# HumanCompatibleAI/imitation

Measured on AMD Instinct MI355X. Metric: env-steps/sec (gen+disc round) GAIL HalfCheetah n_envs=1024, higher is better.
Workload: dtype f32

## Files before the change

imitation_amd/csrc/policy.hip:

```cpp
#include "common.h"
#include "rn_common.h"
#include <algorithm>
#include <type_traits>
#include <cstring>

#include "../../include/imitation_hip.h"
#include "policy_common.h"

namespace {


template <int H>
struct Lds {
  static constexpr int XS = MAXD + 1, HS = H + 1, AS = MAXA + 1;
  static constexpr int x = 0;
  static constexpr int a1 = x + ROWS * XS;
  static constexpr int a2 = a1 + ROWS * HS;
  static constexpr int dz = a2 + ROWS * HS;
  static constexpr int out = dz + ROWS * HS;
  static constexpr int dout = out + ROWS * AS;
  static constexpr int aux = dout + ROWS * AS;
  static constexpr int total = aux + ROWS * AS + 64;
};

// ... 1446 lines not shown
        tr(o.pW1, H, D); tr(o.pW2, H, H); tr(o.vW1, H, D); tr(o.vW2, H, H);
        Pt[dst] = pn;
      }
    }
  }
  if (next_batch > 0 && !stats_block) {
    __syncthreads();
    prepare_stats(d, obs, adv, next_idx, next_batch, T, n_envs, update_norm, nm, nv, ncount, w.advstat, lds);
  }
}

struct CLds {
  static constexpr int RS = 68;
  static constexpr int x = 0;
  static constexpr int a1 = x + MAXD * RS;
  static constexpr int a2 = a1 + 2 * 32 * RS;
  static constexpr int dz2 = a2 + 2 * 32 * RS;
  static constexpr int dz1 = dz2 + 2 * 32 * RS;
  static constexpr int dout = dz1 + 2 * 32 * RS;
  static constexpr int aux = dout + MAXA * RS;
  static constexpr int misc = aux + MAXA * RS;
  static constexpr int scratch = misc + 8 * RS;
  static constexpr int total = scratch + 64;
};


#ifndef IA_UPD_TSTR
#define IA_UPD_TSTR 36
#endif
constexpr int UPD_TSTR = IA_UPD_TSTR;
__host__ __device__ inline int upd_tbase(int off) { return (off * UPD_TSTR + 31) >> 5; }
__host__ __device__ inline int upd_pt4(int P4) { return (upd_tbase(P4) + 3) & ~3; }

template <bool SMALL>
__device__ __forceinline__ void chain_stage_rows(const ia_policy_desc& d, const float* __restrict__ nm,
                                                 const float* __restrict__ nv, const int i0, const int row_lim,
                                                 float* __restrict__ lds, const float* __restrict__ stg, const int tw,
                                                 const int q, const int lane) {
  using L = CLds;
  const int D = d.obs_dim;
  const int S1 = (D + 3) >> 2;
#ifndef IA_SMALL_STAGE_ASIDE
#define IA_SMALL_STAGE_ASIDE 1
#endif
  constexpr int QS = (SMALL && IA_SMALL_STAGE_ASIDE) ? 1 : 0;
  const bool idle = SMALL && q != QS;
  if (!idle) {
    const int rbase = SMALL ? 0 : q * 16;
    const int l128 = lane + 64 * tw;
    const int s1r = (65536 + S1 - 1) / S1;
    for (int g = l128; g < 16 * S1; g += 128) {
      const int r = (g * s1r) >> 16, k0 = (g - r * S1) * 4;
      const bool rok = (i0 + rbase + r) < row_lim;
      float raw[4], mu[4], vr[4];
      {
        const f32x4 rq = *reinterpret_cast<const f32x4*>(stg + UpdStage::x + (rbase * S1 + g) * 4);
        const f32x4 mq = *reinterpret_cast<const f32x4*>(nm + k0);
        const f32x4 vq = *reinterpret_cast<const f32x4*>(nv + k0);
#pragma unroll
        for (int j = 0; j < 4; ++j) {
          raw[j] = rq[j];
          mu[j] = mq[j];
          vr[j] = vq[j];
        }
      }
#pragma unroll
      for (int j = 0; j < 4; ++j) {
        const bool ok = rok && k0 + j < D;
        const bool nrm = ok && d.has_norm;
        lds[L::x + (k0 + j) * L::RS + rbase + r] = ok ? (nrm ? (raw[j] - mu[j]) * vr[j] : raw[j]) : 0.f;
      }
    }
    if (tw == 0) {
      for (int e = lane; e < 16 * MAXA; e += 64) {
        lds[L::dout + (e >> 4) * L::RS + rbase + (e & 15)] = 0.f;
        lds[L::aux + (e >> 4) * L::RS + rbase + (e & 15)] = 0.f;
      }
    } else {
      for (int e = lane; e < 16 * 8; e += 64) lds[L::misc + (e >> 4) * L::RS + rbase + (e & 15)] = 0.f;
    }
  }
}

template <int KS1, bool LOCAL, bool SMALL = false, bool STAGED = false, bool TSPLIT = false>
__device__ __forceinline__ void mfma32_minibatch_chain(
    const ia_policy_desc& d, const float* __restrict__ nm, const float* __restrict__ nv, const float adv_mean,
    const float adv_std, const MbRows rows, const int i0_in, const int row_lim, const int normalize_adv, const float clip,
    const float ent_coef, const float vf_coef, float* __restrict__ slab_g, float* __restrict__ statpart,
    float* __restrict__ lds_in, const float* __restrict__ sP_in, float* __restrict__ stg_in,
    const int opaque_zero, long long* __restrict__ tstamp, const unsigned ll_seq, const bool ll_xcd = false,
    const int split_tw = 0) {
  static_assert(!TSPLIT || (!LOCAL && !SMALL && STAGED), "one tower per workgroup: several gradient workgroups only");
  float* __restrict__ lds = lds_in + opaque_zero;
  const float* __restrict__ stg = stg_in + opaque_zero;
  float* __restrict__ slab = LOCAL ? stg_in + opaque_zero + UpdStage::x : slab_g;
  unsigned long long* __restrict__ slab64 = reinterpret_cast<unsigned long long*>(slab_g);
  auto put = [&](float* p, float v) {
    if constexpr (LOCAL) *p = v;
    else if (ll_xcd) ll_store_xcd(slab64 + (p - slab), v, ll_seq);
    else ll_store_agent(slab64 + (p - slab), v, ll_seq);
  };
  const int batch = rows.batch;
  constexpr int H = 32;
  using L = CLds;
#define IA_TS(slot) do { if (tstamp && i0_in == 0 && threadIdx.x == 0) tstamp[slot] = clock64(); } while (0)
  const int tid = threadIdx.x + opaque_zero, lane = tid & 63;
  const int wv = __builtin_amdgcn_readfirstlane(tid >> 6);
  const int tw = TSPLIT ? split_tw : (SMALL ? (wv & 1) : (wv >> 2)), q = SMALL ? (wv >> 1) : (wv & 3);
  const bool helper = TSPLIT && wv >= 4;
  const int li = lane & 15, lk = lane >> 4;
  const int D = d.obs_dim, A = d.act_dim;
  const PolOff o = pol_offsets(D, A, H, d.discrete);
  const int i0 = i0_in;
  const int aw = d.discrete ? 1 : A;
  const float invB = 1.f / (float)batch;
  const int S1 = (D + 3) >> 2;
  const int oW1 = tw ? o.vW1 : o.pW1, ob1 = tw ? o.vb1 : o.pb1, oW2 = tw ? o.vW2 : o.pW2, ob2 = tw ? o.vb2 : o.pb2;
  const float* __restrict__ sP = sP_in + opaque_zero;
  const float* __restrict__ sPt = sP + ((o.total + 3) & ~3);
  constexpr int TS_ = UPD_TSTR;
  const int tW1 = upd_tbase(oW1), tW2 = upd_tbase(oW2);
  IA_TS(0);

  const int lrow = q * 16 + (lane & 15);
  const bool valid = (i0 + lrow) < row_lim;
  float r_oldlp = 0.f, r_adv = 0.f, r_ret = 0.f, r_act[4] = {0.f, 0.f, 0.f, 0.f};
  constexpr bool HANDOVER = SMALL;
  if (helper) {
  } else if (tw == 0) {
    r_oldlp = stg[UpdStage::oldlp + lrow];
    if constexpr (!HANDOVER) r_adv = stg[UpdStage::adv + lrow];
#pragma unroll
    for (int j = 0; j < 4; ++j) r_act[j] = stg[UpdStage::act + lrow * aw + min(4 * (lane >> 4) + j, aw - 1)];
  } else {
    r_ret = stg[UpdStage::ret + lrow];
    if constexpr (HANDOVER) r_adv = stg[UpdStage::adv + lrow];
  }
  float* gconst = lds + L::scratch + 32;

  IA_TS(9);
  const bool idle = (SMALL && q > 0) || helper;
  if constexpr (!STAGED) chain_stage_rows<SMALL>(d, nm, nv, i0, row_lim, lds, stg, tw, q, lane);
  IA_TS(10);
  constexpr int KT1 = KS1 / 4;
  float fW1[KT1][2][4], fW2[2][2][4], fW2T[2][2][4], fHead[2][4], fHeadT[2][4], b1c[2][4], b2c[2][4], hb[4];
  const int head_base = tw == 0 ? o.aW + min(li, A - 1) * H : o.cW;
  float c_ivar[4] = {1.f, 1.f, 1.f, 1.f}, c_logsd[4] = {0.f, 0.f, 0.f, 0.f};
  if (!helper) {
#pragma unroll
  for (int kt = 0; kt < KT1; ++kt) {
    if (4 * kt < S1) {
#pragma unroll
      for (int t = 0; t < 2; ++t)
#pragma unroll
        for (int r = 0; r < 4; ++r) fW1[kt][t][r] = sPt[tW1 + min(16 * kt + 4 * lk + r, D - 1) * TS_ + 16 * t + li];
    } else {
#pragma unroll
      for (int t = 0; t < 2; ++t)
#pragma unroll
        for (int r = 0; r < 4; ++r) fW1[kt][t][r] = 0.f;
    }
  }
#pragma unroll
  for (int t = 0; t < 2; ++t)
#pragma unroll
    for (int r = 0; r < 4; ++r) b1c[t][r] = sP[ob1 + 16 * t + 4 * lk + r];
  float my_sd = sP[o.log_std + min(lane, A - 1)];
  __builtin_amdgcn_sched_barrier(0);
#pragma unroll
  for (int kt = 0; kt < KT1; ++kt)
#pragma unroll
    for (int t = 0; t < 2; ++t)
#pragma unroll
      for (int r = 0; r < 4; ++r) fW1[kt][t][r] = (16 * kt + 4 * lk + r < D) ? fW1[kt][t][r] : 0.f;
  if constexpr (HANDOVER) {
    if (tw != 0) {
      if (!idle) {
        float advn = r_adv;
        if (normalize_adv && batch > 1) advn = (advn - adv_mean) / (adv_std + 1e-8f);
        if (lk == 0) stg_in[opaque_zero + UpdStage::adv + lrow] = advn;
      }
      if (q == 0 && !d.discrete) {
        const float sd = expf(my_sd);
        const float my_ivar = lane < A ? 1.f / (sd * sd) : 1.f;
        const float my_logsd = lane < A ? logf(sd) : 0.f;
        if (lane < 16) {
          gconst[lane] = my_ivar;
          gconst[16 + lane] = my_logsd;
        }
      }
    }
  } else {
    float my_ivar = 1.f, my_logsd = 0.f;
    if (tw == 0 && !d.discrete) {
      const float sd = expf(my_sd);
      my_ivar = lane < A ? 1.f / (sd * sd) : 1.f;
      my_logsd = lane < A ? logf(sd) : 0.f;
    }
#pragma unroll
    for (int j = 0; j < 4; ++j) {
      c_ivar[j] = __shfl(my_ivar, 4 * lk + j, 64);
      c_logsd[j] = __shfl(my_logsd, 4 * lk + j, 64);
    }
  }
  }
  IA_TS(11);
  __syncthreads();
  IA_TS(1);

  float* a1t = lds + L::a1 + tw * 32 * L::RS;
  float* a2t = lds + L::a2 + tw * 32 * L::RS;
  float* dz2t = lds + L::dz2 + tw * 32 * L::RS;
  float* dz1t = lds + L::dz1 + tw * 32 * L::RS;
  const int trow = 4 * lk * L::RS + q * 16 + li;
  auto xchg16 = [](float v, float& a, float& b) {
    const auto p2 = __builtin_amdgcn_permlane16_swap(__float_as_uint(v), __float_as_uint(v), false, false);
    a = __uint_as_float(p2[0]);
    b = __uint_as_float(p2[1]);
  };
  auto xchg32 = [](float v, float& a, float& b) {
    const auto p2 = __builtin_amdgcn_permlane32_swap(__float_as_uint(v), __float_as_uint(v), false, false);
    a = __uint_as_float(p2[0]);
    b = __uint_as_float(p2[1]);
  };
  auto group_sum = [&](float v) {
    float a, b;
    xchg16(v, a, b);
    v = a + b;
    xchg32(v, a, b);
    return a + b;
  };
  auto group_max = [&](float v) {
    float a, b;
    xchg16(v, a, b);
    v = fmaxf(a, b);
    xchg32(v, a, b);
    return fmaxf(a, b);
  };
  if (!idle) {
  f32x4 a1[2], a2[2];
  {
    f32x4 acc[2][2] = {{{b1c[0][0], b1c[0][1], b1c[0][2], b1c[0][3]}, {0.f, 0.f, 0.f, 0.f}},
                       {{b1c[1][0], b1c[1][1], b1c[1][2], b1c[1][3]}, {0.f, 0.f, 0.f, 0.f}}};
    float xb[KT1][4];
#pragma unroll
    for (int kt = 0; kt < KT1; ++kt)
#pragma unroll
      for (int r = 0; r < 4; ++r) xb[kt][r] = lds[L::x + min(16 * kt + 4 * lk + r, MAXD - 1) * L::RS + q * 16 + li];
    if (HANDOVER && tw == 0) {
      r_adv = stg_in[opaque_zero + UpdStage::adv + lrow];
#pragma unroll
      for (int j = 0; j < 4; ++j) {
        c_ivar[j] = gconst[4 * lk + j];
        c_logsd[j] = gconst[16 + 4 * lk + j];
      }
    }
    __builtin_amdgcn_sched_barrier(0);
#pragma unroll
    for (int kt = 0; kt < KT1; ++kt)
      if (4 * kt < S1) {
#pragma unroll
        for (int r = 0; r < 4; ++r) {
          acc[0][kt & 1] = mfma16(fW1[kt][0][r], xb[kt][r], acc[0][kt & 1]);
          acc[1][kt & 1] = mfma16(fW1[kt][1][r], xb[kt][r], acc[1][kt & 1]);
        }
      }
#pragma unroll
    for (int kt = 0; kt < 2; ++kt)
#pragma unroll
      for (int r = 0; r < 4; ++r)
#pragma unroll
        for (int t = 0; t < 2; ++t) fW2[kt][t][r] = sPt[tW2 + (16 * kt + 4 * lk + r) * TS_ + 16 * t + li];
#pragma unroll
    for (int t = 0; t < 2; ++t)
#pragma unroll
      for (int r = 0; r < 4; ++r) b2c[t][r] = sP[ob2 + 16 * t + 4 * lk + r];
#pragma unroll
    for (int t = 0; t < 2; ++t)
#pragma unroll
      for (int r = 0; r < 4; ++r) {
        a1[t][r] = fast_tanh(acc[t][0][r] + acc[t][1][r]);
        a1t[trow + (16 * t + r) * L::RS] = a1[t][r];
      }
  }
  IA_TS(2);
  {
    f32x4 acc[2][2] = {{{b2c[0][0], b2c[0][1], b2c[0][2], b2c[0][3]}, {0.f, 0.f, 0.f, 0.f}},
                       {{b2c[1][0], b2c[1][1], b2c[1][2], b2c[1][3]}, {0.f, 0.f, 0.f, 0.f}}};
#pragma unroll
    for (int kt = 0; kt < 2; ++kt)
#pragma unroll
      for (int r = 0; r < 4; ++r) {
        acc[0][kt] = mfma16(fW2[kt][0][r], a1[kt][r], acc[0][kt]);
        acc[1][kt] = mfma16(fW2[kt][1][r], a1[kt][r], acc[1][kt]);
      }
    {
      const bool head_on = tw == 0 ? li < A : li == 0;
      float hraw[2][4], braw[4];
#pragma unroll
      for (int kt = 0; kt < 2; ++kt)
#pragma unroll
        for (int r = 0; r < 4; ++r) hraw[kt][r] = sP[head_base + 16 * kt + 4 * lk + r];
#pragma unroll
      for (int r = 0; r < 4; ++r) braw[r] = sP[tw == 0 ? o.ab + min(4 * lk + r, A - 1) : o.cb];
      __builtin_amdgcn_sched_barrier(0);
#pragma unroll
      for (int kt = 0; kt < 2; ++kt)
#pragma unroll
        for (int r = 0; r < 4; ++r) fHead[kt][r] = head_on ? hraw[kt][r] : 0.f;
#pragma unroll
      for (int r = 0; r < 4; ++r) hb[r] = (tw == 0 && 4 * lk + r >= A) ? 0.f : braw[r];
    }
#pragma unroll
    for (int t = 0; t < 2; ++t)
#pragma unroll
      for (int r = 0; r < 4; ++r) {
        a2[t][r] = fast_tanh(acc[t][0][r] + acc[t][1][r]);
        a2t[trow + (16 * t + r) * L::RS] = a2[t][r];
      }
  }
  IA_TS(3);
  float hout[4];
  {
    f32x4 acc[2] = {{hb[0], hb[1], hb[2], hb[3]}, {0.f, 0.f, 0.f, 0.f}};
#pragma unroll
    for (int kt = 0; kt < 2; ++kt)
#pragma unroll
      for (int r = 0; r < 4; ++r) acc[kt] = mfma16(fHead[kt][r], a2[kt][r], acc[kt]);
#pragma unroll
    for (int r = 0; r < 4; ++r) hout[r] = acc[0][r] + acc[1][r];
  }
  IA_TS(4);
#pragma unroll
  for (int kt = 0; kt < 2; ++kt)
#pragma unroll
    for (int t = 0; t < 2; ++t)
#pragma unroll
      for (int r = 0; r < 4; ++r) fW2T[kt][t][r] = sP[oW2 + (16 * kt + 4 * lk + r) * H + 16 * t + li];
#pragma unroll
  for (int t = 0; t < 2; ++t)
#pragma unroll
    for (int r = 0; r < 4; ++r)
      fHeadT[t][r] = sP[tw == 0 ? o.aW + min(4 * lk + r, A - 1) * H + 16 * t + li : o.cW + 16 * t + 4 * lk + r];
  float dout[4] = {0.f, 0.f, 0.f, 0.f}, dvb = 0.f;
  if (tw == 0) {
    float logp = 0.f, entropy = 0.f, lse = 0.f;
    int act_i = 0;
    if (d.discrete) act_i = (int)r_act[0];
    IA_TS(12);
    if (!d.discrete) {
#pragma unroll
      for (int j = 0; j < 4; ++j)
        if (4 * lk + j < A) {
          const float diff = r_act[j] - hout[j];
          logp += -(diff * diff) * (0.5f * c_ivar[j]) - c_logsd[j] - LOG_SQRT_2PI;
          entropy += 0.5f + LOG_SQRT_2PI + c_logsd[j];
        }
      logp = group_sum(logp);
      entropy = group_sum(entropy);
    } else {
      float mx = -3.0e38f, o_act = 0.f;
#pragma unroll
      for (int j = 0; j < 4; ++j)
        if (4 * lk + j < A) {
          mx = fmaxf(mx, hout[j]);
          o_act += (4 * lk + j == act_i) ? hout[j] : 0.f;
        }
      mx = group_max(mx);
      o_act = group_sum(o_act);
      float se = 0.f;
#pragma unroll
      for (int j = 0; j < 4; ++j)
        if (4 * lk + j < A) se += expf(hout[j] - mx);
      lse = mx + logf(group_sum(se));
      logp = o_act - lse;
#pragma unroll
      for (int j = 0; j < 4; ++j)
        if (4 * lk + j < A) {
          const float l = hout[j] - lse;
          entropy -= expf(l) * l;
        }
      entropy = group_sum(entropy);
    }
    IA_TS(13);
    float advn = r_adv;
    if constexpr (!HANDOVER)
      if (normalize_adv && batch > 1) advn = (advn - adv_mean) / (adv_std + 1e-8f);
    const float log_ratio = logp - r_oldlp;
    const float ratio = expf(log_ratio);
    const float lo = 1.f - clip, hi = 1.f + clip;
    const float pl1 = advn * ratio;
    const float pl2 = advn * fminf(fmaxf(ratio, lo), hi);
    const float g1 = pl1 < pl2 ? 1.f : (pl1 == pl2 ? 0.5f : 0.f);
    const float g2 = pl2 < pl1 ? 1.f : (pl1 == pl2 ? 0.5f : 0.f);
    const float inrange = (ratio >= lo && ratio <= hi) ? 1.f : 0.f;
    const float dlogp = valid ? -invB * advn * (g1 + g2 * inrange) * ratio : 0.f;
    IA_TS(14);
    float* doutrow = lds + L::dout + lrow;
    float* auxrow = lds + L::aux + lrow;
    if (!d.discrete) {
#pragma unroll
      for (int j = 0; j < 4; ++j)
        if (4 * lk + j < A) {
          const float diff = r_act[j] - hout[j];
          dout[j] = dlogp * diff * c_ivar[j];
          doutrow[(4 * lk + j) * L::RS] = dout[j];
          auxrow[(4 * lk + j) * L::RS] = valid ? dlogp * (diff * diff * c_ivar[j] - 1.f) - ent_coef * invB : 0.f;
        }
    } else {
#pragma unroll
      for (int j = 0; j < 4; ++j)
        if (4 * lk + j < A) {
          const float l = hout[j] - lse, p = expf(l);
          const float dH = -p * (l + entropy);
          float g = dlogp * ((4 * lk + j == act_i ? 1.f : 0.f) - p);
          g += valid ? -ent_coef * invB * dH : 0.f;
          dout[j] = g;
          doutrow[(4 * lk + j) * L::RS] = g;
        }
    }
    if (lk == 0) {
      float* mrow = lds + L::misc + lrow;
      mrow[2 * L::RS] = valid ? -fminf(pl1, pl2) : 0.f;
      mrow[3 * L::RS] = valid ? -entropy : 0.f;
      mrow[4 * L::RS] = valid ? (ratio - 1.f) - log_ratio : 0.f;
      mrow[5 * L::RS] = valid ? (fabsf(ratio - 1.f) > clip ? 1.f : 0.f) : 0.f;
    }
    IA_TS(15);
  } else {
    const float v = __shfl(hout[0], li, 64);
    const float verr = r_ret - v;
    dvb = valid ? vf_coef * 2.f * (v - r_ret) * invB : 0.f;
    if (lk == 0) {
      lds[L::misc + 1 * L::RS + lrow] = dvb;
      lds[L::misc + 6 * L::RS + lrow] = valid ? verr * verr : 0.f;
    }
  }
  IA_TS(5);
  f32x4 dz2[2];
  if (tw == 0) {
    f32x4 acc[2] = {{0.f, 0.f, 0.f, 0.f}, {0.f, 0.f, 0.f, 0.f}};
#pragma unroll
    for (int r = 0; r < 4; ++r)
      if (r < A) {
        const bool on = 4 * lk + r < A;
        acc[0] = mfma16(on ? fHeadT[0][r] : 0.f, dout[r], acc[0]);
        acc[1] = mfma16(on ? fHeadT[1][r] : 0.f, dout[r], acc[1]);
      }
#pragma unroll
    for (int t = 0; t < 2; ++t)
#pragma unroll
      for (int r = 0; r < 4; ++r) dz2[t][r] = acc[t][r] * (1.f - a2[t][r] * a2[t][r]);
  } else {
#pragma unroll
    for (int t = 0; t < 2; ++t)
#pragma unroll
      for (int r = 0; r < 4; ++r) dz2[t][r] = fHeadT[t][r] * dvb * (1.f - a2[t][r] * a2[t][r]);
  }
#pragma unroll
  for (int t = 0; t < 2; ++t)
#pragma unroll
    for (int r = 0; r < 4; ++r) dz2t[trow + (16 * t + r) * L::RS] = dz2[t][r];
  {
    f32x4 acc[2][2] = {{{0.f, 0.f, 0.f, 0.f}, {0.f, 0.f, 0.f, 0.f}}, {{0.f, 0.f, 0.f, 0.f}, {0.f, 0.f, 0.f, 0.f}}};
#pragma unroll
    for (int kt = 0; kt < 2; ++kt)
#pragma unroll
      for (int r = 0; r < 4; ++r) {
        acc[0][kt] = mfma16(fW2T[kt][0][r], dz2[kt][r], acc[0][kt]);
// ... 2077 lines not shown
      if (tid == 0) ll_store_agent(sq64 + (seq_out & 1u) * 64 + bid, part, seq_out);
    }
    EP_TS(2);
    if (have_next) stage_rows(bnext);
    if (tid < 64) {
      const u64* wp = sq64 + (seq_out & 1u) * 64 + min(tid, nwg - 1);
      u64 t;
      unsigned it = 0;
      for (;;) {
        t = __hip_atomic_load(wp, __ATOMIC_RELAXED, __HIP_MEMORY_SCOPE_AGENT);
        if (__all((unsigned)(t >> 32) == seq_out)) break;
        if (timed_out(it)) { fail = true; break; }
      }
      s_part[tid] = tid < nwg ? __uint_as_float((unsigned)t) : 0.f;
    }
    if (__any(fail) && lane == 0) s_fail = 1;
    __syncthreads();
    if (s_fail) return;
    EP_TS(3);
    float total_sq = 0.f;
    for (int q = 0; q < nwg; ++q) total_sq += s_part[q];
    const float total_norm = sqrtf(total_sq);
    const float coef = fminf(max_norm / (total_norm + 1e-6f), 1.0f);
    {
      const float step_size = st.step_size[k], bc2_sqrt = st.bc2_sqrt[k];
      u64* dst = par64 + (long long)(seq_out & 1u) * o.total;
#pragma unroll
      for (int j = 0; j < NPC; ++j) {
        const int i = i0 + tid + j * NT;
        if (i < i1) {
          const float gi = g[j] * coef;
          const float mi = m_[j] + (gi - m_[j]) * (1.f - beta1);
          const float vi = v_[j] * beta2 + (1.f - beta2) * gi * gi;
          const float denom = sqrtf(vi) / bc2_sqrt + eps;
          const float pn = p_[j] - step_size * (mi / denom);
          ll_store_agent(dst + i, pn, seq_out);
          p_[j] = pn;
          m_[j] = mi;
          v_[j] = vi;
        }
      }
    }
    if (bid == 0 && stats != nullptr) {
      __shared__ float s_st[5];
      if (tid >= 64 && tid < 69) {
        const int kk = tid - 64;
        float sv = 0.f;
        for (int q = 0; q < nblk; ++q) sv += s_stat[q * 8 + kk];
        sv *= 1.f / (float)b;
        stats[(long long)mb * 8 + kk] = sv;
        s_st[kk] = sv;
      }
      __syncthreads();
      if (tid == 0) {
        stats[(long long)mb * 8 + 5] = s_st[0] + ent_coef * s_st[2] + vf_coef * s_st[1];
        stats[(long long)mb * 8 + 6] = total_norm;
        stats[(long long)mb * 8 + 7] = coef;
      }
    }
    EP_TS(4);
  }
  tid = threadIdx.x;
#pragma unroll
  for (int j = 0; j < NPC; ++j) {
    const int i = bid * chunk + tid + j * NT;
    if (i < min(o.total, (bid + 1) * chunk)) {
      m[i] = m_[j];
      v[i] = v_[j];
      P[i] = p_[j];
      int dst = i;
      auto tr = [&](int b0, int rows_, int cols) {
        if (i >= b0 && i < b0 + rows_ * cols) {
          const int r = (i - b0) / cols, cc = (i - b0) % cols;
          dst = b0 + cc * rows_ + r;
        }
      };
      tr(o.pW1, H, D); tr(o.pW2, H, H); tr(o.vW1, H, D); tr(o.vW2, H, H);
      Pt[dst] = p_[j];
    }
  }
#undef EP_TS
}

template <int NPT, bool TIMING, int KS1, bool LOCAL, bool SHARD, bool SMALL, bool TSPLIT, int OWNER>
__device__ __forceinline__ void ppo_update_body(
    const ia_policy_desc& d, float* __restrict__ P, float* __restrict__ Pt, float* __restrict__ m, float* __restrict__ v,
    float* __restrict__ nm, float* __restrict__ nv, int32_t* __restrict__ ncount, int update_norm,
    const float* __restrict__ obs, const float* __restrict__ actions, const float* __restrict__ old_logp,
    const float* __restrict__ adv, const float* __restrict__ ret, const int64_t* __restrict__ perm, int T, int n_envs,
    int normalize_adv, float clip, float ent_coef, float vf_coef, float max_norm, float beta1, float beta2, float eps,
    float* __restrict__ ws, int nblk, int n_slices, float* __restrict__ stats, UpdSched sch, int xcd_pack,
    long long* __restrict__ tstamp ,
    ShardArgs sh) {
  constexpr int H = 32;
  using L = CLds;
  extern __shared__ float lds_raw[];
  float* lds = lds_raw + (((16u - (__builtin_amdgcn_groupstaticsize() & 15u)) & 15u) >> 2);
  __shared__ int s_ok, s_pub, s_fail, s_pubw[4];
  if (!TIMING) tstamp = nullptr;
  long long tacc[12] = {0, 0, 0, 0, 0, 0, 0, 0, 0, 0, 0, 0};
  long long tprev = 0, tend = 0;
#define UPD_TS(k) do { if (tstamp && tid == 0) { const long long tn = wall_clock64(); tacc[k] += tn - tprev; tprev = tn; } } while (0)
  if (xcd_pack && (blockIdx.x & 7)) return;
  const int vb = xcd_pack ? blockIdx.x >> 3 : blockIdx.x;
  static_assert(!TSPLIT || (!LOCAL && !SHARD && !SMALL), "one tower per workgroup: several gradient workgroups, one process");
  static_assert(OWNER == 0 || (OWNER == 1 && TSPLIT), "slices by tower: the tower-split form only");
  const int ngw = TSPLIT ? 2 * nblk : nblk;
  const int rb = TSPLIT ? vb >> 1 : vb;
  const int split_tw = TSPLIT ? (vb & 1) : 0;
  const int tid = threadIdx.x;
  const int D = d.obs_dim;
  const PolOff o = pol_offsets(D, d.act_dim, H, d.discrete);
  const UpdWs w = upd_ws(ws, nblk, o.total);
  unsigned* arrivals = w.ctrl + 64;
  unsigned* published = w.ctrl + 1;
  unsigned* sliced = w.ctrl + 16;
  unsigned* err = w.ctrl + 8;
  const unsigned lseq_base = __hip_atomic_load(w.ctrl + 9, __ATOMIC_RELAXED, __HIP_MEMORY_SCOPE_AGENT);
  if (threadIdx.x == 0) s_fail = 0;
  bool ll_xcd = false;
  if constexpr (!LOCAL && !TSPLIT) {
    if (xcd_pack && vb < nblk && nblk <= 64) {
      __shared__ int s_xcd;
      unsigned xcc;
      asm volatile("s_getreg_b32 %0, hwreg(HW_REG_XCC_ID)" : "=s"(xcc));
      xcc &= 0xfu;
      const unsigned aseq = ~lseq_base;
      unsigned long long* aw = w.slabs64 + w.P4 + 7;
      const long long P8a = w.P4 + 8;
      if (tid == 0) ll_store_agent(aw + (long long)vb * P8a, __uint_as_float(xcc), aseq);
      if (tid < 64) {
        const unsigned long long* wp = aw + (long long)min(tid, nblk - 1) * P8a;
        unsigned long long t;
        bool bad = false;
        const long long t0a = wall_clock64();
        for (unsigned it = 0;;) {
          t = __hip_atomic_load(wp, __ATOMIC_RELAXED, __HIP_MEMORY_SCOPE_AGENT);
          if (__all((unsigned)(t >> 32) == aseq)) break;
          __builtin_amdgcn_s_sleep(1);
          if ((++it & 255u) == 0 &&
              (__hip_atomic_load(err, __ATOMIC_RELAXED, __HIP_MEMORY_SCOPE_AGENT) || wall_clock64() - t0a > 200000000ll)) {
            bad = true;
            break;
          }
        }
        if (tid == 0) {
          s_xcd = 0;
          if (bad) s_fail = 1;
        }
        if (!bad && __all((unsigned)t == xcc) && tid == 0) s_xcd = 1;
      }
      __syncthreads();
      if (s_fail) {
        if (tid == 0) __hip_atomic_store(err, 1u, __ATOMIC_RELAXED, __HIP_MEMORY_SCOPE_AGENT);
        return;
      }
      ll_xcd = s_xcd != 0;
      if (tstamp && tid == 0 && vb < 8) tstamp[42 + vb] = (long long)xcc * 2 + (ll_xcd ? 1 : 0);
    }
  }

  const int sch_first = sch.first, sch_nmb = sch.n_mb, sch_bs = sch.batch_size, n_steps = sch.n_steps;
  const long long sch_total = sch.total;
  const int row_lo = SHARD ? sh.rank * sh.rows_per_rank : 0;
  auto row_lim = [&](const MbRows& r) { return SHARD ? min(r.batch, row_lo + sh.rows_per_rank) : r.batch; };
  auto rows_at = [=](int e, int mb) {
// ... 139 lines not shown
      __syncthreads();
      if (d.has_norm && tid < D) {
        slot[tid] = nm[tid];
        slot[MAXD + tid] = 1.f / sqrtf(nv[tid] + d.norm_eps);
      }
      __syncthreads();
      if (tid == 0) {
        __threadfence();
        __hip_atomic_store(published, (unsigned)(s + 1), __ATOMIC_RELAXED, __HIP_MEMORY_SCOPE_AGENT);
      }
      SB_TS(2);
    }
    if (tstamp && tid == 0) { tstamp[12] += sb_acc[0]; tstamp[13] += sb_acc[1]; tstamp[14] += sb_acc[2]; }
#undef SB_TS
    if (tid < 64) {
      const bool ok = spin_arrivals(arrivals, (unsigned)n_steps, 1, err);
      if (tid == 0) {
        s_ok = ok;
        __threadfence();
      }
    }
    __syncthreads();
    if (!s_ok) return;
    drain(n_steps - 1);
    return;
  }
  if (vb > ngw) {
    constexpr int NPH = TSPLIT ? 2 : 1;
    const int jj = vb - ngw - 1;
    const int j = jj / NPH;
    if (j >= n_slices) return;
    for (int s = jj - j * NPH; s < n_steps; s += NPH) {
      const MbRows r = rows_of(s);
      const int r0 = j * UPD_SLICE;
      const int nr = min(UPD_SLICE, r.batch - r0);
      if (s >= UPD_RING) {
        if (tid == 0) s_ok = spin_until(published, (unsigned)(s - UPD_RING + 1), err);
        __syncthreads();
        if (!s_ok) return;
      }
      if (nr > 0) {
        float* pj = w.pring + ((long long)(s % UPD_RING) * UPD_SLICES_MAX + j) * UPD_PRS;
        prepare_stats_t<512>(d, r.obs, r.adv, r.idx + r0, nr, T, n_envs, update_norm, nullptr, nullptr, nullptr, nullptr,
                             lds, reinterpret_cast<int*>(lds + PREP_LDS_FLOATS), pj);
      }
      __syncthreads();
      if (tid == 0) {
        __threadfence();
        if (NPH == 1 || s == 0 || spin_until(sliced + j, (unsigned)s, err))
          __hip_atomic_store(sliced + j, (unsigned)(s + 1), __ATOMIC_RELAXED, __HIP_MEMORY_SCOPE_AGENT);
      }
    }
    return;
  }

  constexpr int PROWS = SMALL ? 16 : ROWS;
  float* sP = lds + L::total;
  float* sPt = sP + w.P4;
  float* stg = sPt + upd_pt4(w.P4);
  unsigned short* dstT = reinterpret_cast<unsigned short*>(stg + UpdStage::total(d.discrete ? 1 : d.act_dim));
  const int lane = tid & 63;
  float rm[NPT], rv[NPT];
#pragma unroll
  for (int k = 0; k < NPT; ++k) {
    const int i = tid + k * 512;
    rm[k] = rv[k] = 0.f;
    if (i < o.total) {
      const float pi_ = P[i];
      sP[i] = pi_;
      rm[k] = m[i];
      rv[k] = v[i];
      int dst = 0xffff;
      auto tr = [&](int base, int rows, int cols) {
        if (i >= base && i < base + rows * cols) {
          const int rr = (i - base) / cols, cc = (i - base) % cols;
          dst = upd_tbase(base) + cc * UPD_TSTR + rr;
        }
      };
      tr(o.pW1, H, D); tr(o.pW2, H, H); tr(o.vW1, H, D); tr(o.vW2, H, H);
      dstT[i] = (unsigned short)dst;
      if (dst != 0xffff) sPt[dst] = pi_;
    }
  }
  auto prefetch_resolve = [&](const MbRows& r) {
    if (tid >= 448) {
      int tz;
      asm volatile("s_mov_b32 %0, 0" : "=s"(tz));
      const unsigned Tq = (unsigned)(T + tz);
      const int i0 = row_lo + rb * ROWS;
      int src = 0;
      if (i0 + lane < row_lim(r)) {
        const long long flat = r.idx[i0 + lane];
        if (sch_total < (1ll << 31)) {
          const unsigned f = (unsigned)flat, env = f / Tq, t = f - env * Tq;
          src = (int)(t * (unsigned)n_envs + env);
        } else {
          src = (int)rollout_offset(flat, T, n_envs);
        }
      }
      reinterpret_cast<int*>(stg)[UpdStage::nxt + lane] = src;
    }
  };
  typedef __attribute__((address_space(3))) void* lds_void_p;
  typedef __attribute__((address_space(1))) const void* glb_void_p;
  const int wave = __builtin_amdgcn_readfirstlane(tid >> 6);
  auto prefetch_issue = [&](const MbRows& r, int zero) {
    const int* nxt = reinterpret_cast<const int*>(stg) + UpdStage::nxt;
    constexpr int SCW = 7;
    int src0 = 0;
    if (wave == SCW) src0 = nxt[lane];
    const int Q = (D + 3) >> 2;
    constexpr int NQT = (PROWS * (MAXD / 4) + 511) / 512;
    int qsrc[NQT], qoff[NQT];
    const unsigned rcpQ = 0xffffffffu / (unsigned)Q + 1u;
#pragma unroll
    for (int it = 0; it < NQT; ++it) {
      const int e0 = it * 512 + wave * 64 + zero;
      qsrc[it] = qoff[it] = 0;
      if (e0 < PROWS * Q) {
        const int e = min(e0 + lane, PROWS * Q - 1);
        const int rr = Q == 1 ? e : (int)__umulhi((unsigned)e, rcpQ);
        qoff[it] = 4 * (e - rr * Q);
        qsrc[it] = nxt[rr];
      }
    }
    const int aw_ = d.discrete ? 1 : d.act_dim;
    constexpr int NAT = (PROWS * MAXA + 511) / 512;
    int asrc[NAT], acol[NAT];
    const unsigned rcpA = 0xffffffffu / (unsigned)aw_ + 1u;
#pragma unroll
    for (int it = 0; it < NAT; ++it) {
      const int e0 = it * 512 + wave * 64 + zero;
      acol[it] = asrc[it] = 0;
      if (e0 < PROWS * aw_) {
        const int e = min(e0 + lane, PROWS * aw_ - 1);
        const int rr = aw_ == 1 ? e : (int)__umulhi((unsigned)e, rcpA);
        acol[it] = e - rr * aw_;
        asrc[it] = nxt[rr];
      }
    }
    asm volatile("s_waitcnt lgkmcnt(0)" ::: "memory");
#pragma unroll
    for (int it = 0; it < NQT; ++it) {
      const int e0 = it * 512 + wave * 64;
      if (e0 < PROWS * Q)
        __builtin_amdgcn_global_load_lds((glb_void_p)(r.obs + (long long)qsrc[it] * D + qoff[it]),
                                         (lds_void_p)(stg + UpdStage::x + 4 * e0), 16, 0, 0);
    }
#pragma unroll
    for (int it = 0; it < NAT; ++it) {
      const int e0 = it * 512 + wave * 64;
      if (e0 < PROWS * aw_)
        __builtin_amdgcn_global_load_lds((glb_void_p)(r.actions + (long long)asrc[it] * aw_ + acol[it]),
                                         (lds_void_p)(stg + UpdStage::act + e0), 4, 0, 0);
    }
    if (wave == SCW) {
      __builtin_amdgcn_global_load_lds((glb_void_p)(r.old_logp + src0), (lds_void_p)(stg + UpdStage::oldlp), 4, 0, 0);
      __builtin_amdgcn_global_load_lds((glb_void_p)(r.adv + src0), (lds_void_p)(stg + UpdStage::adv), 4, 0, 0);
      __builtin_amdgcn_global_load_lds((glb_void_p)(r.ret + src0), (lds_void_p)(stg + UpdStage::ret), 4, 0, 0);
    }
  };
  auto prefetch_park = [&]() {
    if (wave == 0) stg[UpdStage::src + lane] = stg[UpdStage::nxt + lane];
    asm volatile("s_waitcnt vmcnt(0)" ::: "memory");
  };
  for (int e = tid; e < (SMALL ? L::total : MAXD * L::RS); e += 512) lds[L::x + e] = 0.f;
  int cur_e = sch_first / sch_nmb, cur_mb = sch_first - cur_e * sch_nmb;
  if (n_steps > 0) {
    prefetch_resolve(rows_at(cur_e, cur_mb));
    __syncthreads();
    prefetch_issue(rows_at(cur_e, cur_mb), 0);
    prefetch_park();
  }
  __syncthreads();

  bool have_ring = false;
  constexpr bool local = LOCAL;
  if (tstamp && tid == 0) tprev = wall_clock64();
  for (int s = 0; s < n_steps; ++s) {
    const MbRows r = rows_at(cur_e, cur_mb);
    const bool wrap = cur_mb + 1 == sch_nmb;
    const int nxt_e = wrap ? cur_e + 1 : cur_e, nxt_mb = wrap ? 0 : cur_mb + 1;
    cur_e = nxt_e;
    cur_mb = nxt_mb;
    const float* slot = w.ring + (s % UPD_RING) * UPD_RS;
    float adv_mean, adv_std;
    if (!have_ring) {
      if (tid == 0) {
        s_ok = spin_until(published, (unsigned)(s + 1), err);
        __threadfence();
      }
      __syncthreads();
      if (!s_ok) return;
      {
        int sz;
        asm volatile("s_mov_b32 %0, 0" : "=s"(sz));
        if (tid < 2 * MAXD + 8) stg[UpdStage::ring + tid] = *reinterpret_cast<const volatile float*>(slot + tid + sz);
      }
      __syncthreads();
      if constexpr (!LOCAL) {
        int zz;
        asm volatile("s_mov_b32 %0, 0" : "=s"(zz));
        const int wv_ = __builtin_amdgcn_readfirstlane((tid + zz) >> 6);
        chain_stage_rows<false>(d, stg + UpdStage::ring, stg + UpdStage::ring + MAXD, row_lo + rb * ROWS, row_lim(r), lds, stg,
                                wv_ >> 2, wv_ & 3, lane);
      }
    }
    slot = stg + UpdStage::ring;
    const int pub_early = (int)__hip_atomic_load(published, __ATOMIC_RELAXED, __HIP_MEMORY_SCOPE_AGENT);
    adv_mean = slot[2 * MAXD];
    adv_std = slot[2 * MAXD + 1];
    UPD_TS(0);
    const float step_size = w.tab[s], bc2_sqrt = w.tab[UPD_MAX_STEPS + s];
    if (s + 1 < n_steps) prefetch_resolve(rows_at(nxt_e, nxt_mb));
    const int P8 = w.P4 + 8;
    const unsigned lseq = lseq_base + (unsigned)s + 1u;
    const int xpar = SHARD ? (int)((sh.seq_base + (unsigned)s) & 1u) : 0;
    unsigned long long* slabs_s = w.slabs64 + (long long)(s & 1) * nblk * P8;
    float* stat_base = w.statpart + (s % UPD_SD) * nblk * 8;
    int oz;
    asm volatile("s_mov_b32 %0, 0" : "=s"(oz));
    mfma32_minibatch_chain<KS1, LOCAL, SMALL, !LOCAL, TSPLIT>(d, slot, slot + MAXD, adv_mean, adv_std, r, row_lo + rb * ROWS, row_lim(r),
                                       normalize_adv, clip, ent_coef, vf_coef,
                                       reinterpret_cast<float*>(slabs_s + (long long)rb * P8), stat_base + vb * 8, lds, sP,
                                       stg, oz, (tstamp && (!TSPLIT || vb == 0)) ? tstamp + 16 : nullptr, lseq, ll_xcd, split_tw);
    UPD_TS(1);
    if constexpr (TSPLIT) {
      if (tstamp && tid == 0) tend += tprev;
    }
    UPD_TS(7);
    UPD_TS(8);
    float g[NPT];
    unsigned long long tail_w = 0ull;
    const bool want_tail = !LOCAL && vb == 0 && tid < 64 && stats;
    if (local) {
      int gz;
      asm volatile("s_mov_b32 %0, 0" : "=s"(gz));
#pragma unroll
      for (int k = 0; k < NPT; ++k) g[k] = stg[UpdStage::x + gz + min(tid + k * 512, o.total - 1)];
      if constexpr (SHARD) asm volatile("s_waitcnt vmcnt(0)" ::: "memory");
      if (tid == 0) {
        s_ok = 1;
        s_pub = pub_early;
        asm volatile("buffer_inv sc1" ::: "memory");
      }
      __syncthreads();
    }
    if (s + 1 < n_steps) {
      int pz;
      asm volatile("s_mov_b32 %0, 0" : "=s"(pz));
      prefetch_issue(rows_at(nxt_e, nxt_mb), pz);
    }
    if constexpr (!LOCAL) {
      if (s + 1 < n_steps && wave < 3) {
        if (pub_early >= s + 2) {
          const float* nslot = w.ring + ((s + 1) % UPD_RING) * UPD_RS;
          __builtin_amdgcn_global_load_lds((glb_void_p)(nslot + wave * MAXD + lane),
                                           (lds_void_p)(stg + UpdStage::ring + wave * MAXD), 4, 0, 0);
        }
        if (lane == 0) s_pubw[wave] = pub_early;
      }
    }
    UPD_TS(9);
    if constexpr (LOCAL) {
      UPD_TS(10);
      UPD_TS(11);
    } else {
      using u64 = unsigned long long;
      const int SL = (P8 + ngw - 1) / ngw;
      const unsigned rcpSL = 0xffffffffu / (unsigned)SL + 1u;
      float* red = lds + L::a1;
      auto valid_el = [&](int gi) { return gi < o.total || (gi >= w.P4 && gi < w.P4 + 5); };
      bool fail = false;
      const long long t0 = wall_clock64();
      const long long local_timeout = 200000000ll;
      u64* sums_s = w.sums64 + (long long)(s & 1) * P8;
      auto emit = [&](int gi, float part) {
        if constexpr (SHARD) {
          const unsigned xseq = sh.seq_base + (unsigned)s + 1u;
          for (int rr = 0; rr < sh.world; ++rr)
            ll_store_system(sh.peer_recv[rr] + (long long)(xpar * sh.world + (sh.loopback ? rr : sh.rank)) * P8 + gi, part, xseq);
        } else if (ll_xcd) {
          ll_store_xcd(sums_s + gi, part, lseq);
        } else {
          ll_store_agent(sums_s + gi, part, lseq);
        }
      };
      if constexpr (OWNER == 0) {
      {
      {
        u64 t[NPT];
        int gi_[NPT];
        unsigned need = 0u;
        int ez;
        asm volatile("s_mov_b32 %0, 0" : "=s"(ez));
#pragma unroll
        for (int k = 0; k < NPT; ++k) {
          const int f = tid + ez + k * 512;
          const int j = (int)__umulhi((unsigned)f, rcpSL), e = f - j * SL;
          const int gi = vb * SL + e;
          gi_[k] = min(j, nblk - 1) * P8 + min(gi, P8 - 1);
          if (f < nblk * SL && valid_el(gi)) need |= 1u << k;
        }
        unsigned it = 0;
        for (;; ) {
// ... 271 lines not shown
            break;
          }
        }
#pragma unroll
        for (int u = 0; u < SHARD_RB; ++u)
          if (r0 + u < W) {
#pragma unroll
            for (int k = 0; k < NPT; ++k) g[k] += __uint_as_float((unsigned)t[u][k]);
          }
      }
      if (fail) {
        __hip_atomic_store(err, 2u, __ATOMIC_RELAXED, __HIP_MEMORY_SCOPE_AGENT);
        s_ok = 0;
      }
      __syncthreads();
      if (!s_ok) return;
    }
#pragma unroll
    for (int k = 0; k < NPT; ++k) {
      if (tid + k * 512 >= o.total) g[k] = 0.f;
      sq += g[k] * g[k];
    }
    UPD_TS(4);
    int rz;
    asm volatile("s_mov_b32 %0, 0" : "=s"(rz));
    const float total_sq = block_sum512_dpp(sq, lds + L::scratch + rz, s & 1);
    if constexpr (!LOCAL) {
      if (s_fail) {
        if (tid == 0) __hip_atomic_store(err, SHARD ? 2u : 1u, __ATOMIC_RELAXED, __HIP_MEMORY_SCOPE_AGENT);
        return;
      }
      have_ring = (s + 1 < n_steps) && (s_pub >= s + 2);
    }
    UPD_TS(5);
    const float total_norm = sqrtf(total_sq);
    const float coef = fminf(max_norm / (total_norm + 1e-6f), 1.0f);
    if constexpr (!LOCAL) {
      if (vb == 0 && tid < 64 && stats) {
        const float st = __uint_as_float((unsigned)tail_w) * (1.f / (float)r.batch);
        const float st0 = __shfl(st, 0, 64), st1 = __shfl(st, 1, 64), st2 = __shfl(st, 2, 64);
        float* so = stats + (long long)(sch_first + s) * 8;
        if (lane < 5) so[lane] = st;
        if (lane == 5) so[5] = st0 + ent_coef * st2 + vf_coef * st1;
        if (lane == 6) so[6] = total_norm;
        if (lane == 7) so[7] = coef;
      }
    } else if constexpr (SHARD) {
      if (vb == 0 && tid < 64 && stats) {
        const unsigned long long* rbase = sh.recv + (long long)(xpar * sh.world) * (w.P4 + 8) + w.P4;
        const unsigned seq = sh.seq_base + (unsigned)s + 1u;
        const int rk = min(lane >> 3, sh.world - 1);
        unsigned long long tv;
        const long long t0 = wall_clock64();
        bool late = false;
        do {
          tv = __hip_atomic_load(rbase + rk * (w.P4 + 8) + (lane & 7), __ATOMIC_RELAXED, __HIP_MEMORY_SCOPE_SYSTEM);
          late = !__all((unsigned)(tv >> 32) == seq);
        } while (late && wall_clock64() - t0 < sh.timeout_ticks);
        if (late && lane == 0)
          __hip_atomic_store(err, 2u, __ATOMIC_RELAXED, __HIP_MEMORY_SCOPE_AGENT);
        float st = (lane >> 3) < sh.world ? __uint_as_float((unsigned)tv) : 0.f;
        {
          float acc = __shfl(st, lane & 7, 64);
          for (int r_ = 1; r_ < sh.world; ++r_) acc += __shfl(st, r_ * 8 + (lane & 7), 64);
          st = acc * (1.f / (float)r.batch);
        }
        const float st0 = __shfl(st, 0, 64), st1 = __shfl(st, 1, 64), st2 = __shfl(st, 2, 64);
        float* so = stats + (long long)(sch_first + s) * 8;
        if (lane < 5) so[lane] = st;
        if (lane == 5) so[5] = st0 + ent_coef * st2 + vf_coef * st1;
        if (lane == 6) so[6] = total_norm;
        if (lane == 7) so[7] = coef;
      }
    } else if (vb == 0) {
      if (s + 1 < n_steps) {
        if (tid == 0) {
          slab_store(w.normcoef + (s % UPD_SD) * 2, total_norm);
          slab_store(w.normcoef + (s % UPD_SD) * 2 + 1, coef);
        }
      } else {
        write_loss_stats(s, total_norm, coef);
      }
    }
    {
      float pv[NPT];
      int dt[NPT];
#pragma unroll
      for (int k = 0; k < NPT; ++k) {
        const int ic = min(tid + k * 512, o.total - 1);
        pv[k] = sP[ic];
        dt[k] = dstT[ic];
      }
      __builtin_amdgcn_sched_barrier(0);
      const float inv_bc2 = 1.f / bc2_sqrt;
#pragma unroll
      for (int k = 0; k < NPT; ++k) {
        const float gi = g[k] * coef;
        float mi = rm[k];
        mi = mi + (gi - mi) * (1.f - beta1);
        const float vi = rv[k] * beta2 + (1.f - beta2) * gi * gi;
        const float denom = __builtin_amdgcn_sqrtf(vi) * inv_bc2 + eps;
        float rd = __builtin_amdgcn_rcpf(denom);
        rd = __builtin_fmaf(rd, __builtin_fmaf(-denom, rd, 1.f), rd);
        pv[k] = pv[k] - step_size * (mi * rd);
        rm[k] = mi;
        rv[k] = vi;
      }
      __builtin_amdgcn_sched_barrier(0);
#pragma unroll
      for (int k = 0; k < NPT; ++k) {
        const int i = tid + k * 512;
        if (i < o.total) {
          sP[i] = pv[k];
          if (dt[k] != 0xffff) sPt[dt[k]] = pv[k];
        }
      }
    }
    UPD_TS(6);
    if (s + 1 < n_steps && (LOCAL || !have_ring)) prefetch_park();
    else if (local) asm volatile("s_waitcnt vmcnt(0)" ::: "memory");
    __syncthreads();
    if (local && tid == 0)
      __hip_atomic_fetch_add(arrivals + 16 * (vb & (UPD_ARR - 1)), 1u, __ATOMIC_RELAXED, __HIP_MEMORY_SCOPE_AGENT);
    UPD_TS(3);
  }
#undef UPD_TS
  if (tstamp && vb == 0 && tid == 0)
    for (int k = 0; k < 12; ++k) tstamp[k] += tacc[k];
  if constexpr (TSPLIT) {
    if (tstamp && vb == 1 && tid == 0)
      for (int k = 0; k < 12; ++k) tstamp[50 + k] += tacc[k];
    if (tstamp && vb < 2 && tid == 0) tstamp[62 + vb] += tend;
  }
  if (vb == 0 && tid == 0)
    __hip_atomic_store(w.ctrl + 9, lseq_base + (unsigned)n_steps, __ATOMIC_RELAXED, __HIP_MEMORY_SCOPE_AGENT);
  if (vb == 0) {
#pragma unroll
    for (int k = 0; k < NPT; ++k) {
      const int i = tid + k * 512;
      if (i < o.total) {
        const float pi_ = sP[i];
        P[i] = pi_;
        int dst = i;
        auto tr = [&](int base, int rows, int cols) {
          if (i >= base && i < base + rows * cols) {
            const int rr = (i - base) / cols, cc = (i - base) % cols;
            dst = base + cc * rows + rr;
          }
        };
        tr(o.pW1, H, D); tr(o.pW2, H, H); tr(o.vW1, H, D); tr(o.vW2, H, H);
        Pt[dst] = pi_;
        m[i] = rm[k];
        v[i] = rv[k];
      }
    }
  }
}

#define IA_UPD_KERNEL_PARAMS                                                                                              \
  ia_policy_desc d, float *__restrict__ P, float *__restrict__ Pt, float *__restrict__ m, float *__restrict__ v,         \
      float *__restrict__ nm, float *__restrict__ nv, int32_t *__restrict__ ncount, int update_norm,                     \
      const float *__restrict__ obs, const float *__restrict__ actions, const float *__restrict__ old_logp,              \
      const float *__restrict__ adv, const float *__restrict__ ret, const int64_t *__restrict__ perm, int T, int n_envs, \
      int normalize_adv, float clip, float ent_coef, float vf_coef, float max_norm, float beta1, float beta2, float eps, \
      float *__restrict__ ws, int nblk, int n_slices, float *__restrict__ stats, UpdSched sch, int xcd_pack,             \
      long long *__restrict__ tstamp, ShardArgs sh
#define IA_UPD_KERNEL_ARGS                                                                                               \
  d, P, Pt, m, v, nm, nv, ncount, update_norm, obs, actions, old_logp, adv, ret, perm, T, n_envs, normalize_adv, clip,    \
      ent_coef, vf_coef, max_norm, beta1, beta2, eps, ws, nblk, n_slices, stats, sch, xcd_pack, tstamp, sh

template <int NPT, bool TIMING, int KS1, bool LOCAL, bool SHARD = false, bool SMALL = false>
__global__ __launch_bounds__(512) void ppo_update_persistent_kernel(IA_UPD_KERNEL_PARAMS) {
  ppo_update_body<NPT, TIMING, KS1, LOCAL, SHARD, SMALL, false, 0>(IA_UPD_KERNEL_ARGS);
}

template <int NPT, bool TIMING, int KS1>
__global__ __launch_bounds__(512) void ppo_update_split_kernel(IA_UPD_KERNEL_PARAMS) {
  ppo_update_body<NPT, TIMING, KS1, false, false, false, true, 0>(IA_UPD_KERNEL_ARGS);
}
template <int NPT, bool TIMING, int KS1>
__global__ __launch_bounds__(512) void ppo_update_owner_kernel(IA_UPD_KERNEL_PARAMS) {
  ppo_update_body<NPT, TIMING, KS1, false, false, false, true, 1>(IA_UPD_KERNEL_ARGS);
}
#undef IA_UPD_KERNEL_PARAMS
#undef IA_UPD_KERNEL_ARGS

inline int cdiv(long long a, long long b) { return (int)((a + b - 1) / b); }

template <int H>
size_t lds_bytes() { return Lds<H>::total * sizeof(float); }

struct LaunchSlot {
  size_t lds_set = 0;
  int per_cu = -1;
  size_t per_cu_lds = 0;
};

template <typename K>
int ensure_lds(LaunchSlot& s, K kern, size_t bytes) {
  if (bytes <= s.lds_set) return IA_OK;
  hipError_t e = hipFuncSetAttribute(reinterpret_cast<const void*>(kern), hipFuncAttributeMaxDynamicSharedMemorySize,
                                     (int)bytes);
  if (e != hipSuccess) return (int)e;
  s.lds_set = bytes;
  return IA_OK;
}

int device_cus() {
  static int cus = 0;
  if (cus == 0) {
    int dev = 0, n = 0;
    if (hipGetDevice(&dev) != hipSuccess ||
        hipDeviceGetAttribute(&n, hipDeviceAttributeMultiprocessorCount, dev) != hipSuccess)
      return 0;
    cus = n;
  }
  return cus;
}

template <typename K>
int fits_resident(LaunchSlot& s, K kern, int threads, size_t bytes, long long grid, int cus) {
  if (s.per_cu < 0 || s.per_cu_lds != bytes) {
    int nb = 0;
// ... 793 lines not shown
```

Measured before the change: 4.943 million.

## Offload loss constants to helper waves and split Adam update by tower ownership

```diff
diff --git a/imitation_amd/csrc/policy.hip b/imitation_amd/csrc/policy.hip
--- a/imitation_amd/csrc/policy.hip
+++ b/imitation_amd/csrc/policy.hip
@@ -1552,7 +1552,10 @@
   }
 }
 
-template <int KS1, bool LOCAL, bool SMALL = false, bool STAGED = false, bool TSPLIT = false>
+#ifndef IA_UPD_HELPER_CONSTS
+#define IA_UPD_HELPER_CONSTS 1
+#endif
+template <int KS1, bool LOCAL, bool SMALL = false, bool STAGED = false, bool TSPLIT = false, bool HCONST = false>
 __device__ __forceinline__ void mfma32_minibatch_chain(
     const ia_policy_desc& d, const float* __restrict__ nm, const float* __restrict__ nv, const float adv_mean,
     const float adv_std, const MbRows rows, const int i0_in, const int row_lim, const int normalize_adv, const float clip,
@@ -1561,6 +1564,7 @@
     const int opaque_zero, long long* __restrict__ tstamp, const unsigned ll_seq, const bool ll_xcd = false,
     const int split_tw = 0) {
   static_assert(!TSPLIT || (!LOCAL && !SMALL && STAGED), "one tower per workgroup: several gradient workgroups only");
+  static_assert(!HCONST || TSPLIT, "loss constants from the helper waves: the tower-split form only");
   float* __restrict__ lds = lds_in + opaque_zero;
   const float* __restrict__ stg = stg_in + opaque_zero;
   float* __restrict__ slab = LOCAL ? stg_in + opaque_zero + UpdStage::x : slab_g;
@@ -1597,9 +1601,11 @@
   float r_oldlp = 0.f, r_adv = 0.f, r_ret = 0.f, r_act[4] = {0.f, 0.f, 0.f, 0.f};
   constexpr bool HANDOVER = SMALL;
   if (helper) {
+    if constexpr (HCONST)
+      if (tw == 0) r_adv = stg[UpdStage::adv + lrow];
   } else if (tw == 0) {
     r_oldlp = stg[UpdStage::oldlp + lrow];
-    if constexpr (!HANDOVER) r_adv = stg[UpdStage::adv + lrow];
+    if constexpr (!HANDOVER && !HCONST) r_adv = stg[UpdStage::adv + lrow];
 #pragma unroll
     for (int j = 0; j < 4; ++j) r_act[j] = stg[UpdStage::act + lrow * aw + min(4 * (lane >> 4) + j, aw - 1)];
   } else {
@@ -1660,7 +1666,7 @@
         }
       }
     }
-  } else {
+  } else if constexpr (!HCONST) {
     float my_ivar = 1.f, my_logsd = 0.f;
     if (tw == 0 && !d.discrete) {
       const float sd = expf(my_sd);
@@ -1673,6 +1679,21 @@
       c_logsd[j] = __shfl(my_logsd, 4 * lk + j, 64);
     }
   }
+  } else if constexpr (HCONST) {
+    if (tw == 0) {
+      float advn = r_adv;
+      if (normalize_adv && batch > 1) advn = (advn - adv_mean) / (adv_std + 1e-8f);
+      if (lk == 0) stg_in[opaque_zero + UpdStage::adv + lrow] = advn;
+      if (q == 0 && !d.discrete) {
+        const float sd = expf(sP[o.log_std + min(lane, A - 1)]);
+        const float my_ivar = lane < A ? 1.f / (sd * sd) : 1.f;
+        const float my_logsd = lane < A ? logf(sd) : 0.f;
+        if (lane < 16) {
+          gconst[lane] = my_ivar;
+          gconst[16 + lane] = my_logsd;
+        }
+      }
+    }
   }
   IA_TS(11);
   __syncthreads();
@@ -1717,7 +1738,7 @@
     for (int kt = 0; kt < KT1; ++kt)
 #pragma unroll
       for (int r = 0; r < 4; ++r) xb[kt][r] = lds[L::x + min(16 * kt + 4 * lk + r, MAXD - 1) * L::RS + q * 16 + li];
-    if (HANDOVER && tw == 0) {
+    if ((HANDOVER || HCONST) && tw == 0) {
       r_adv = stg_in[opaque_zero + UpdStage::adv + lrow];
 #pragma unroll
       for (int j = 0; j < 4; ++j) {
@@ -1854,7 +1875,7 @@
     }
     IA_TS(13);
     float advn = r_adv;
-    if constexpr (!HANDOVER)
+    if constexpr (!HANDOVER && !HCONST)
       if (normalize_adv && batch > 1) advn = (advn - adv_mean) / (adv_std + 1e-8f);
     const float log_ratio = logp - r_oldlp;
     const float ratio = expf(log_ratio);
@@ -4098,6 +4119,9 @@
 #undef EP_TS
 }
 
+#ifndef IA_UPD_OWN_TOWER_ADAM
+#define IA_UPD_OWN_TOWER_ADAM 1
+#endif
 template <int NPT, bool TIMING, int KS1, bool LOCAL, bool SHARD, bool SMALL, bool TSPLIT, int OWNER>
 __device__ __forceinline__ void ppo_update_body(
     const ia_policy_desc& d, float* __restrict__ P, float* __restrict__ Pt, float* __restrict__ m, float* __restrict__ v,
@@ -4403,6 +4427,16 @@
       if (dst != 0xffff) sPt[dst] = pi_;
     }
   }
+  constexpr bool OWNT = TSPLIT && OWNER == 0 && IA_UPD_OWN_TOWER_ADAM;
+  unsigned ownm = 0u;
+  if constexpr (OWNT) {
+#pragma unroll
+    for (int k = 0; k < NPT; ++k) {
+      const int i = tid + k * 512;
+      const bool pol = i < o.vW1 || (i >= o.aW && i < o.cW);
+      if (i < o.total && pol == (split_tw == 0)) ownm |= 1u << k;
+    }
+  }
   auto prefetch_resolve = [&](const MbRows& r) {
     if (tid >= 448) {
       int tz;
@@ -4541,7 +4575,7 @@
     float* stat_base = w.statpart + (s % UPD_SD) * nblk * 8;
     int oz;
     asm volatile("s_mov_b32 %0, 0" : "=s"(oz));
-    mfma32_minibatch_chain<KS1, LOCAL, SMALL, !LOCAL, TSPLIT>(d, slot, slot + MAXD, adv_mean, adv_std, r, row_lo + rb * ROWS, row_lim(r),
+    mfma32_minibatch_chain<KS1, LOCAL, SMALL, !LOCAL, TSPLIT, TSPLIT && OWNER == 0 && IA_UPD_HELPER_CONSTS != 0>(d, slot, slot + MAXD, adv_mean, adv_std, r, row_lo + rb * ROWS, row_lim(r),
                                        normalize_adv, clip, ent_coef, vf_coef,
                                        reinterpret_cast<float*>(slabs_s + (long long)rb * P8), stat_base + vb * 8, lds, sP,
                                        stg, oz, (tstamp && (!TSPLIT || vb == 0)) ? tstamp + 16 : nullptr, lseq, ll_xcd, split_tw);
@@ -4979,7 +5013,50 @@
         write_loss_stats(s, total_norm, coef);
       }
     }
-    {
+    if constexpr (OWNT) {
+      int az;
+      asm volatile("s_mov_b32 %0, 0" : "=s"(az));
+      const unsigned om = ownm + (unsigned)az;
+      unsigned wm = 0u;
+#pragma unroll
+      for (int k = 0; k < NPT; ++k)
+        if (__builtin_amdgcn_ballot_w64(((om >> k) & 1u) != 0u) != 0ull) wm |= 1u << k;
+      float pv[NPT];
+      int dt[NPT];
+#pragma unroll
+      for (int k = 0; k < NPT; ++k) {
+        pv[k] = 0.f;
+        dt[k] = 0xffff;
+        if ((wm >> k) & 1u) {
+          const int ic = min(tid + k * 512, o.total - 1);
+          pv[k] = sP[ic];
+          dt[k] = dstT[ic];
+        }
+      }
+      __builtin_amdgcn_sched_barrier(0);
+      const float inv_bc2 = 1.f / bc2_sqrt;
+#pragma unroll
+      for (int k = 0; k < NPT; ++k)
+        if ((wm >> k) & 1u) {
+          const float gi = g[k] * coef;
+          float mi = rm[k];
+          mi = mi + (gi - mi) * (1.f - beta1);
+          const float vi = rv[k] * beta2 + (1.f - beta2) * gi * gi;
+          const float denom = __builtin_amdgcn_sqrtf(vi) * inv_bc2 + eps;
+          float rd = __builtin_amdgcn_rcpf(denom);
+          rd = __builtin_fmaf(rd, __builtin_fmaf(-denom, rd, 1.f), rd);
+          pv[k] = pv[k] - step_size * (mi * rd);
+          rm[k] = mi;
+          rv[k] = vi;
+        }
+      __builtin_amdgcn_sched_barrier(0);
+#pragma unroll
+      for (int k = 0; k < NPT; ++k)
+        if ((om >> k) & 1u) {
+          sP[tid + k * 512] = pv[k];
+          if (dt[k] != 0xffff) sPt[dt[k]] = pv[k];
+        }
+    } else {
       float pv[NPT];
       int dt[NPT];
 #pragma unroll
@@ -5031,11 +5108,11 @@
   }
   if (vb == 0 && tid == 0)
     __hip_atomic_store(w.ctrl + 9, lseq_base + (unsigned)n_steps, __ATOMIC_RELAXED, __HIP_MEMORY_SCOPE_AGENT);
-  if (vb == 0) {
+  if (OWNT ? vb < 2 : vb == 0) {
 #pragma unroll
     for (int k = 0; k < NPT; ++k) {
       const int i = tid + k * 512;
-      if (i < o.total) {
+      if (OWNT ? ((ownm >> k) & 1u) != 0u : i < o.total) {
         const float pi_ = sP[i];
         P[i] = pi_;
         int dst = i;
```

Result: slower. 4.878 million (-1.3%).
